# ChristodoulosPappas/IPLS-Java-API

Hardware: AMD Instinct MI355X
Metric: aggregated-gradient GB/s (device-resident), 32 peers×4M doubles/partition (higher is better)
Workload: dtype f64

## Files before the change

### include/ipls_agg.h

```cpp
#ifndef IPLS_AGG_H
#define IPLS_AGG_H

#include <stddef.h>
#include <stdint.h>

#ifdef __cplusplus
extern "C" {
#endif

#define IPLS_AGG_ABI_VERSION 4

#define IPLS_OK           0
#define IPLS_E_INVAL     -1
#define IPLS_E_RANGE     -2
#define IPLS_E_NEGSIZE   -3
#define IPLS_E_NOMEM     -4
#define IPLS_E_DEVICE    -5
#define IPLS_E_FORMAT    -6
#define IPLS_E_NODEV     -7

#define IPLS_TGT_AGG      0
#define IPLS_TGT_REP      1
#define IPLS_TGT_WEIGHTS  2
#define IPLS_TGT_WADDR    3
// ... 180 lines not shown
#define IPLS_KERNEL_REDUCE        1
#define IPLS_KERNEL_ROUND         2
#define IPLS_KERNEL_FOLD1         3
#define IPLS_KERNEL_REDUCE_SCALAR 4
#define IPLS_KERNEL_REDUCE_F32    5
#define IPLS_KERNEL_REDUCE_H16    6
#define IPLS_KERNEL_ROUND_F32     7
#define IPLS_KERNEL_ROUND_H16     8
#define IPLS_KERNEL_FOLD1_F32     9
#define IPLS_KERNEL_FOLD1_H16    10
#define IPLS_KERNEL_UPDATE_FLAT  11
#define IPLS_SHAPE_BIG    1
#define IPLS_SHAPE_MID    2
#define IPLS_SHAPE_SMALL  3
#define IPLS_SHAPE_HALF   4
typedef struct ipls_launch_info {
    int32_t kernel, shape, block, vectors, seqf, map;
    int64_t grid;
    int32_t be_in, be_out, start;
    int32_t staged;
} ipls_launch_info;
int ipls_agg_last_launch(ipls_agg *h, ipls_launch_info *out);


int ipls_host_alloc(size_t bytes, void **ptr);
int ipls_host_free(void *ptr);


int ipls_synth_fill(void *dst, int64_t len, uint64_t seed, int p, int k, int dst_kind,
                    void *stream);

int ipls_checksum_dev(const void *src, int64_t n, int src_kind, uint64_t *out, void *stream);

int ipls_encode_secure(const void *src, void *dst, int64_t n, int src_kind, int dst_kind,
                       void *stream);

int64_t ipls_frame_parse(const uint8_t *frame, int64_t len, int16_t *pid, int32_t *a,
                         int32_t *b, int64_t *payload_off, int64_t *origin_off);

int64_t ipls_frame_encode(const double *g, int64_t n, int g_kind, int32_t a, int32_t b,
                          int16_t pid, const uint8_t *origin, int32_t origin_len,
                          uint8_t *out, int64_t out_cap);


int64_t ipls_pair_parse(const uint8_t *buf, int64_t len, int32_t *workers, int64_t *payload_off);

// ... 35 lines not shown
```

### ipls-java-api_amd/csrc/engine.hip

```cpp
#include <hip/hip_runtime.h>

#include <algorithm>
#include <atomic>
#include <cstdarg>
#include <cstdio>
#include <cstdlib>
#include <cstring>
#include <deque>
#include <map>
#include <memory>
#include <mutex>
#include <new>
#include <set>
#include <string>
#include <thread>
#include <vector>

#include "../../include/ipls_agg.h"
#include "ipls_kernels.hpp"
#include "javaser.hpp"
#include "engine.hpp"
#include "pubsub_host.hpp"

using namespace ipls;
// ... 30 lines not shown
  hipEvent_t free_ev = nullptr;
  bool free_pending = false;
};

struct ipls_dev {
  std::mutex mu;
  std::string err;
  int device = 0;
  hipStream_t stream = nullptr;

  int64_t model_size = 0;
  int P = 0;
  int64_t chunk = 0;
  int secure = 0;
  std::vector<int64_t> len, flat_off;
  int64_t max_len = 0, flat_total = 0;
  int p_lo = 0;
  int64_t flat_base = 0;

  double* arena = nullptr;
  int64_t arena_elems = 0;
  std::vector<int64_t> agg_off, rep_off, w_off, fut_off;
  std::vector<uint8_t> agg_zero, rep_zero, fut_zero;

  PinnedSlot ring[kRingSlots];
  void* d_table[kRingSlots] = {};
  size_t d_table_cap[kRingSlots] = {};
  int ring_next = 0;
  std::vector<unsigned char> last_table;
  int last_slot = -1;

  std::mutex stage_mu;
  std::vector<ipls_stage*> stage_all, stage_idle;
  void* d_scratch = nullptr;
  size_t scratch_bytes = 0;
  hipEvent_t copy_ev = nullptr;
  static constexpr int kCopyThreads = 4;
  hipStream_t copy_stream[kCopyThreads] = {};
  hipEvent_t ingest_ev = nullptr;
  std::vector<hipEvent_t> msg_ev;
  struct StageSlot {
    void* d = nullptr;
    size_t cap = 0;
    hipEvent_t free_ev = nullptr;
    bool pending = false;
  };
// ... 66 lines not shown
int check_part(ipls_dev* h, int p) {
  if (p < 0 || p >= h->P) return fail(h, IPLS_E_RANGE, "partition %d out of range [0,%d)", p, h->P);
  return IPLS_OK;
}

int64_t target_off(ipls_dev* h, int p, int target) {
  switch (target) {
    case IPLS_TGT_AGG: return h->agg_off[p];
    case IPLS_TGT_REP: return h->rep_off[p];
    case IPLS_TGT_WEIGHTS:
    case IPLS_TGT_WADDR: return h->w_off[p];
    case IPLS_TGT_FUTURE: return h->fut_off[p];
    default: return -1;
  }
}

uint8_t* zero_flag(ipls_dev* h, int p, int target) {
  if (target == IPLS_TGT_AGG) return &h->agg_zero[p];
  if (target == IPLS_TGT_REP) return &h->rep_zero[p];
  if (target == IPLS_TGT_FUTURE) return &h->fut_zero[p];
  return nullptr;
}

int materialize(ipls_dev* h, int p, int target) {
  uint8_t* f = zero_flag(h, p, target);
  if (f && *f) {
    HIP_TRY(h, hipMemsetAsync(h->arena + target_off(h, p, target), 0, (size_t)h->len[p] * 8, h->stream));
    *f = 0;
  }
  return IPLS_OK;
}

int ensure_pinned(ipls_dev* h, PinnedSlot& s, size_t bytes) {
  if (s.pending) {
    HIP_TRY(h, hipEventSynchronize(s.ev));
    s.pending = false;
  }
  if (s.cap < bytes) {
    if (s.host) HIP_TRY(h, hipHostFree(s.host));
    s.host = nullptr;
    s.cap = 0;
    size_t cap = std::max<size_t>(bytes, 64 << 10);
    HIP_TRY(h, hipHostMalloc(&s.host, cap, hipHostMallocDefault));
    s.cap = cap;
  }
  if (!s.ev) HIP_TRY(h, hipEventCreateWithFlags(&s.ev, hipEventDisableTiming));
  return IPLS_OK;
}

int fail_nl(ipls_dev* h, int code, const char* fmt, ...) {
  char buf[512];
// ... 535 lines not shown
    if (nz == n_parts) start = IPLS_START_ZERO;
    else if (nz) {
      for (int q = 0; q < n_parts; ++q) {
        int rc = materialize(h, p_first + q, target);
        if (rc) return rc;
      }
    }
  }
  if (!fin && !tr_in && n_parts == 1 && k == 1 && bufs[0]) {
    unsigned long long* d0 = dst_of(0);
    const int64_t L = len_of(0);
    if (d0 && !((uintptr_t)bufs[0] & 15) && !((uintptr_t)d0 & 15) && L > 0) {
      const auto* s0 = (const unsigned long long*)bufs[0];
      const unsigned blocks =
          std::max(1u, std::min<unsigned>(blocks_for((L >> 1), kBlock * 4), host_src ? 128u : 4096u));
#define F1(BI, BO, ST) hipLaunchKernelGGL((k_fold1<BI, BO, ST>), dim3(blocks), dim3(kBlock), 0, h->stream, d0, s0, L)
#define F1S(BI, BO) do { if (start == kZero) F1(BI, BO, kZero); else if (start == kFirst) F1(BI, BO, kFirst); else F1(BI, BO, kAccum); } while (0)
      if (be_in) { if (be_out) F1S(true, true); else F1S(true, false); }
      else { if (be_out) F1S(false, true); else F1S(false, false); }
#undef F1S
#undef F1
      HIP_TRY(h, hipGetLastError());
      h->last_launch = launch_info(IPLS_KERNEL_FOLD1, 0, kBlock, 4, 0, 0, blocks, be_in, be_out, kstart(start));
      if (!ext_dst)
        if (uint8_t* f = zero_flag(h, p_first, target)) *f = 0;
      return IPLS_OK;
    }
  }
  if (!fin && tr_in && arrival && !be_out && start != IPLS_START_FIRST && n_parts == 1 && k == 1 && bufs[0]) {
    unsigned long long* d0 = dst_of(0);
    const int64_t L = len_of(0);
    if (d0 && !((uintptr_t)bufs[0] & (uintptr_t)(4 * fmt_size(fmt_in) - 1)) && !((uintptr_t)d0 & 15) && L > 0) {
      const unsigned blocks = std::max(1u, std::min<unsigned>(blocks_for(L >> 2, kBlock * kFold1NarrowR), kFold1NarrowGrid));
      with_narrow(fmt_in, [&](auto s) {
        typedef decltype(s) S;
        const auto* s0 = (const typename S::elem*)bufs[0];
        if (start == IPLS_START_ZERO)
          hipLaunchKernelGGL((k_fold1_narrow<S, kZero, kFold1NarrowR>), dim3(blocks), dim3(kBlock), 0, h->stream, d0, s0, L);
        else
          hipLaunchKernelGGL((k_fold1_narrow<S, kAccum, kFold1NarrowR>), dim3(blocks), dim3(kBlock), 0, h->stream, d0, s0, L);
      });
      HIP_TRY(h, hipGetLastError());
      h->last_launch = launch_info(fmt_size(fmt_in) == 4 ? IPLS_KERNEL_FOLD1_F32 : IPLS_KERNEL_FOLD1_H16, 0, kBlock,
                                   kFold1NarrowR, 1, 0, blocks, false, false, kstart(start));
      if (!ext_dst)
        if (uint8_t* f = zero_flag(h, p_first, target)) *f = 0;
      return IPLS_OK;
    }
  }
  bool aligned16 = true;
  int64_t maxL = 0;
  for (int q = 0; q < n_parts; ++q) maxL = std::max(maxL, len_of(q));
  for (int64_t i = 0; i < (int64_t)n_parts * k; ++i) {
    if (!bufs[i]) return fail(h, IPLS_E_INVAL, "bucket pointer %lld is NULL", (long long)i);
    uintptr_t a = (uintptr_t)bufs[i];
    if (a & (uintptr_t)(fmt_size(fmt_in) - 1))
      return fail(h, IPLS_E_INVAL, "bucket %lld not %d-byte aligned", (long long)i, fmt_size(fmt_in));
    if (a & 15) aligned16 = false;
  }
  const size_t desc_bytes = sizeof(PartDesc) * n_parts;
  const size_t bytes = desc_bytes + sizeof(void*) * (size_t)n_parts * k;
  std::vector<unsigned char> tbl(bytes);
  PartDesc* pd = (PartDesc*)tbl.data();
  for (int q = 0; q < n_parts; ++q) {
    const int p = p_first + q;
    pd[q].len = len_of(q);
    pd[q].dst = dst_of(q);
    pd[q].init = pd[q].dst;
    pd[q].rep = nullptr;
// ... 31 lines not shown
    }
    HIP_TRY(h, hipGetLastError());
    for (int q = p_first; q < p_first + n_parts; ++q) h->agg_zero[q] = h->rep_zero[q] = 1;
    return IPLS_OK;
  }
  if (tr_in) {
    h->last_launch = with_narrow(fmt_in, [&](auto s) {
      typedef decltype(s) S;
      return launch_reduce_narrow<S>(be_out, kstart(start), aligned16, maxL, n_parts, h->stream,
                                     (const typename S::elem* const*)dbufs, dparts, k);
    });
  } else if (aligned16) {
    h->last_launch = launch_reduce(be_in, be_out, start, maxL, n_parts, h->stream, dbufs, dparts, k);
  } else {
    const int64_t tile = (int64_t)kBlock * 8;
    const int tpp = (int)((maxL + tile - 1) / tile);
    launch_reduce_scalar(be_in, be_out, start, dim3((unsigned)tpp * n_parts), h->stream, dbufs, dparts, k, tpp,
                         tile);
    h->last_launch = launch_info(IPLS_KERNEL_REDUCE_SCALAR, 0, kBlock, 1, 0, 0, (int64_t)tpp * n_parts, be_in, be_out,
                                 kstart(start));
  }
  HIP_TRY(h, hipGetLastError());
  if (!ext_dst)
    for (int q = 0; q < n_parts; ++q) {
      uint8_t* f = zero_flag(h, p_first + q, target);
      if (f) *f = 0;
    }
  return IPLS_OK;
}

int partition_geometry(const ipls_agg_cfg* c, std::vector<int64_t>& len, std::vector<int64_t>& off,
                       int64_t& chunk, std::string& why) {
  const int P = c->n_partitions;
  len.resize(P);
  off.resize(P);
  if (c->model_size > 0) {
    chunk = ref_chunk(c->model_size, P);
    for (int i = 0; i < P; ++i) {
      int64_t L = ((int64_t)(i + 1) * chunk > c->model_size) ? c->model_size - (int64_t)i * chunk + 1
                                                             : chunk + 1;
      if (L < 1) {
        char b[160];
        snprintf(b, sizeof b, "partition %d length %lld < 1 (%s)", i, (long long)L,
                 L < 0 ? "NegativeArraySizeException, IPLS.java:1863"
                       : "ArrayIndexOutOfBoundsException, IPLS.java:1894");
        why = b;
        return L < 0 ? IPLS_E_NEGSIZE : IPLS_E_RANGE;
      }
      len[i] = L;
      off[i] = (int64_t)i * chunk;
// ... 52 lines not shown
  if (!h) return fail(nullptr, IPLS_E_NOMEM, "host allocation failed");
  std::string why;
  std::vector<int64_t> glen, goff;
  int rc = partition_geometry(cfg, glen, goff, h->chunk, why);
  if (rc) {
    delete h;
    return fail(nullptr, rc, "%s", why.c_str());
  }
  h->len.assign(glen.begin() + p_lo, glen.begin() + p_hi);
  h->flat_off.assign(goff.begin() + p_lo, goff.begin() + p_hi);
  h->p_lo = p_lo;
  h->flat_base = p_hi > p_lo ? h->flat_off[0] : 0;
  h->P = p_hi - p_lo;
  h->device = device;
  h->model_size = cfg->model_size;
  h->secure = cfg->secure;
  h->agg_off.resize(h->P);
  h->rep_off.resize(h->P);
  h->w_off.resize(h->P);
  h->fut_off.resize(h->P);
  h->agg_zero.assign(h->P, 1);
  h->rep_zero.assign(h->P, 1);
  h->fut_zero.assign(h->P, 1);
  int64_t cur = 0;
  for (int p = 0; p < h->P; ++p) {
    h->max_len = std::max(h->max_len, h->len[p]);
    h->flat_total = std::max(h->flat_total, h->flat_off[p] + h->len[p] - 1);
    h->agg_off[p] = cur; cur = align_up(cur + h->len[p], kAlignElems);
    h->rep_off[p] = cur; cur = align_up(cur + h->len[p], kAlignElems);
    h->w_off[p] = cur;   cur = align_up(cur + h->len[p], kAlignElems);
    h->fut_off[p] = cur; cur = align_up(cur + h->len[p], kAlignElems);
  }
  h->arena_elems = cur;
  h->gbuf_len = h->model_size > 0 ? (int64_t)((int32_t)h->model_size / cfg->n_partitions) + 2 : cfg->bucket_len;
  auto cleanup = [&](int code) {
    (void)hipGetLastError();
    dev_close(h);
    return code;
  };
  if (dev_use(h->device) != hipSuccess) return cleanup(fail(nullptr, IPLS_E_DEVICE, "dev_use(%d) failed", h->device));
  if (hipStreamCreateWithFlags(&h->stream, hipStreamNonBlocking) != hipSuccess)
    return cleanup(fail(nullptr, IPLS_E_DEVICE, "hipStreamCreate failed"));
  if (h->arena_elems > 0 && hipMalloc(&h->arena, (size_t)h->arena_elems * 8) != hipSuccess) {
    (void)hipGetLastError();
    h->arena = nullptr;
    return cleanup(fail(nullptr, IPLS_E_NOMEM, "hipMalloc of %lld-byte arena failed", (long long)h->arena_elems * 8));
// ... 569 lines not shown
            const flat_job& f = fj[j0 + j];
            if (f.q < 0 || f.q >= h->P || f.ncopy < 0 || f.ncopy > h->len[f.q] - 1 || f.lo < 0)
              return fail(h, IPLS_E_INVAL, "internal: bad whole-gradient job");
            FlatJob& o = jobs[(size_t)j];
            o.lo = f.lo;
            o.ncopy = f.ncopy;
            o.L = h->len[f.q];
            o.dst = (unsigned long long*)(h->arena + h->agg_off[f.q]);
            o.zero = h->agg_zero[f.q];
            maxL = std::max(maxL, o.L);
            all_vec = all_vec && f.ncopy >= tile;
            all_zero = all_zero && o.zero;
          }
          void* djobs = nullptr;
          if (int r = upload_table(h, jobs.data(), jobs.size() * sizeof(FlatJob), &djobs)) return r;
          const dim3 grid(blocks_for(maxL, tile), (unsigned)nj);
          if (fmt == kFmtF64) launch_update_flat<FmtD64, false>(h->stream, grid, (const FlatJob*)djobs, d_in);
          else if (fmt == kFmtBE) launch_update_flat<FmtD64, true>(h->stream, grid, (const FlatJob*)djobs, d_in);
          else
            with_narrow(fmt, [&](auto sfmt) {
              launch_update_flat<decltype(sfmt), false>(h->stream, grid, (const FlatJob*)djobs, d_in);
            });
          HIP_TRY(h, hipGetLastError());
          for (int j = 0; j < nj; ++j) h->agg_zero[fj[j0 + j].q] = 0;
          h->last_launch = launch_info(IPLS_KERNEL_UPDATE_FLAT, 0, kBlock, kFlatR, all_vec ? 1 : 0, 0,
                                       (int64_t)grid.x * grid.y, fmt == kFmtBE, false, all_zero ? kZero : kAccum);
        }
      }
      return IPLS_OK;
    }();
  }
  for (int s = 0; s < n; ++s) {
    ipls_dev* h = c[s].h;
    ipls_stage* st = c[s].st;
    if (dev_use(h->device) == hipSuccess && hipEventRecord(st->free_ev, h->stream) == hipSuccess) {
      st->free_pending = true;
    } else {
      (void)hipGetLastError();
      (void)hipStreamSynchronize(h->stream);
      st->free_pending = false;
    }
  }
  for (int s = n - 1; s >= 0; --s) c[s].h->mu.unlock();
  for (int s = 0; s < n; ++s) {
    if (rc) {
      (void)dev_use(c[s].h->device);
      for (int i = 0; i < c[s].st->n_copy; ++i) (void)hipStreamSynchronize(c[s].st->copy[i]);
// ... 155 lines not shown
int dev_reset(ipls_dev* h, int p) {
  if (!h) return fail(nullptr, IPLS_E_INVAL, "null handle");
  IPLS_LOCK(h);
  if (p == IPLS_ALL_PARTITIONS) {
    for (int q = 0; q < h->P; ++q) h->agg_zero[q] = h->rep_zero[q] = 1;
    return IPLS_OK;
  }
  if (int rc = check_part(h, p)) return rc;
  h->agg_zero[p] = h->rep_zero[p] = 1;
  return IPLS_OK;
}

int dev_promote_future(ipls_dev* h, const int32_t* parts, int n_parts) {
  if (!h) return fail(nullptr, IPLS_E_INVAL, "null handle");
  IPLS_LOCK(h);
  if (n_parts < 0 || (n_parts > 0 && !parts)) return fail(h, IPLS_E_INVAL, "bad partition list");
  for (int i = 0; i < n_parts; ++i)
    if (int rc = check_part(h, parts[i])) return rc;
  for (int i = 0; i < n_parts; ++i) {
    const int p = parts[i];
    std::swap(h->agg_off[p], h->fut_off[p]);
    h->agg_zero[p] = h->fut_zero[p];
    h->fut_zero[p] = 1;
  }
  return IPLS_OK;
}

int dev_device_ptr(ipls_dev* h, int p, int target, void** ptr) {
  if (!h || !ptr) return fail(h, IPLS_E_INVAL, "null argument");
  IPLS_LOCK(h);
  if (int rc = check_part(h, p)) return rc;
  if (target_off(h, p, target) < 0) return fail(h, IPLS_E_INVAL, "bad target %d", target);
  HIP_TRY(h, dev_use(h->device));
  if (int rc = materialize(h, p, target)) return rc;
  *ptr = h->arena + target_off(h, p, target);
  return IPLS_OK;
}

int dev_read(ipls_dev* h, int p, int target, void* dst, int64_t n, int dst_kind) {
  if (!h || !dst) return fail(h, IPLS_E_INVAL, "null argument");
  IPLS_LOCK(h);
  if (int rc = check_part(h, p)) return rc;
  if (target_off(h, p, target) < 0) return fail(h, IPLS_E_INVAL, "bad target %d", target);
  const int64_t L = h->len[p];
  if (n < L) return fail(h, IPLS_E_RANGE, "output of %lld < partition length %lld", (long long)n, (long long)L);
  HIP_TRY(h, dev_use(h->device));
  if (int rc = materialize(h, p, target)) return rc;
  const double* srcd = h->arena + target_off(h, p, target);
  switch (dst_kind) {
    case IPLS_HOST_F64:
      return d2h(h, dst, srcd, (size_t)L * 8);
    case IPLS_DEV_F64:
      HIP_TRY(h, hipMemcpyAsync(dst, srcd, (size_t)L * 8, hipMemcpyDeviceToDevice, h->stream));
      return IPLS_OK;
    case IPLS_DEV_BE:
      launch_bswap(h->stream, (const unsigned long long*)srcd, (unsigned long long*)dst, L);
      HIP_TRY(h, hipGetLastError());
      return IPLS_OK;
// ... 8 lines not shown
  }
}

int dev_checksum(ipls_dev* h, int p, int target, uint64_t* out) {
  if (!h || !out) return fail(h, IPLS_E_INVAL, "null argument");
  IPLS_LOCK(h);
  if (int rc = check_part(h, p)) return rc;
  if (target_off(h, p, target) < 0) return fail(h, IPLS_E_INVAL, "bad target %d", target);
  HIP_TRY(h, dev_use(h->device));
  if (int rc = materialize(h, p, target)) return rc;
  HIP_TRY(h, hipMemsetAsync(h->d_sum, 0, 8, h->stream));
  const int64_t L = h->len[p];
  hipLaunchKernelGGL(k_checksum<false>, dim3(std::max(1u, std::min<unsigned>(blocks_for(L, kBlock * 8), 2048))),
                     dim3(kBlock), 0, h->stream,
                     (const unsigned long long*)(h->arena + target_off(h, p, target)), L, h->d_sum);
  HIP_TRY(h, hipGetLastError());
  unsigned long long v = 0;
  if (int rc = d2h(h, &v, h->d_sum, 8)) return rc;
  *out = v;
  return IPLS_OK;
}

static int finalize_range(ipls_dev* h, int p0, int np) {
  bool rep_zero_all = true;
  for (int q = p0; q < p0 + np; ++q) {
    if (int rc = materialize(h, q, IPLS_TGT_AGG)) return rc;
    rep_zero_all = rep_zero_all && h->rep_zero[q];
  }
  if (!rep_zero_all)
    for (int q = p0; q < p0 + np; ++q)
      if (int rc = materialize(h, q, IPLS_TGT_REP)) return rc;
  std::vector<FinDesc> fd(np);
  int64_t maxL = 0;
  for (int q = 0; q < np; ++q) {
    fd[q] = FinDesc{h->len[p0 + q], h->agg_off[p0 + q], h->rep_off[p0 + q], h->w_off[p0 + q]};
    maxL = std::max(maxL, fd[q].len);
  }
  void* dtab = nullptr;
  if (int rc = upload_table(h, fd.data(), fd.size() * sizeof(FinDesc), &dtab)) return rc;
  const int64_t tile = kFinTile;
  const int tpp = (int)((maxL + tile - 1) / tile);
  if (rep_zero_all)
    hipLaunchKernelGGL((k_finalize<true, false>), dim3((unsigned)tpp * np), dim3(kBlock), 0, h->stream,
                       (const FinDesc*)dtab, h->arena, tpp);
  else
    hipLaunchKernelGGL((k_finalize<false, false>), dim3((unsigned)tpp * np), dim3(kBlock), 0, h->stream,
                       (const FinDesc*)dtab, h->arena, tpp);
  HIP_TRY(h, hipGetLastError());
  for (int q = p0; q < p0 + np; ++q) h->agg_zero[q] = h->rep_zero[q] = 1;
  return IPLS_OK;
}

static int divide_range(ipls_dev* h, int p0, int np, unsigned long long* d_out, bool be) {
  std::vector<DivDesc> dd(np);
  int64_t maxn = 0;
  for (int q = 0; q < np; ++q) {
    const int p = p0 + q;
    dd[q] = DivDesc{h->len[p], h->w_off[p], h->flat_off[p] - h->flat_off[p0]};
    maxn = std::max(maxn, h->len[p] - 1);
  }
  if (maxn <= 0) return IPLS_OK;
  void* dtab = nullptr;
  if (int rc = upload_table(h, dd.data(), dd.size() * sizeof(DivDesc), &dtab)) return rc;
  const int64_t tile = kDivTile;
  const int tpp = (int)((maxn + tile - 1) / tile);
  const dim3 g((unsigned)tpp * np);
#define DIV(B, S) hipLaunchKernelGGL((k_divide<B, S>), g, dim3(kBlock), 0, h->stream, (const DivDesc*)dtab, (const double*)h->arena, d_out, tpp)
  if (be) { if (h->secure) DIV(true, true); else DIV(true, false); }
  else { if (h->secure) DIV(false, true); else DIV(false, false); }
#undef DIV
  HIP_TRY(h, hipGetLastError());
  return IPLS_OK;
// ... 484 lines not shown
    const bool vec = al16((const char*)d + esz * lo) && al16(acc);
    const dim3 g = vec ? dim3(std::max(1u, blocks_for(L, kEwTile))) : dim3(blocks_for(L, kBlock));
#define UPD(BI, M)                                                                                              \
  do {                                                                                                          \
    if (vec) hipLaunchKernelGGL((k_split<BI, false, M, true>), g, dim3(kBlock), 0, h->stream, d, lo, nc[p], L, acc); \
    else hipLaunchKernelGGL((k_split<BI, false, M, false>), g, dim3(kBlock), 0, h->stream, d, lo, nc[p], L, acc); \
  } while (0)
#define UPDN(M)                                                                                                 \
  do {                                                                                                          \
    if (vec) hipLaunchKernelGGL((k_split_narrow<S, false, M, true>), g, dim3(kBlock), 0, h->stream, (const typename S::elem*)d, lo, nc[p], L, acc); \
    else hipLaunchKernelGGL((k_split_narrow<S, false, M, false>), g, dim3(kBlock), 0, h->stream, (const typename S::elem*)d, lo, nc[p], L, acc); \
  } while (0)
    if (fmt_trainer(fmt))
      with_narrow(fmt, [&](auto s) {
        typedef decltype(s) S;
        if (zero) UPDN(2);
        else UPDN(1);
      });
    else if (be) { if (zero) UPD(true, 2); else UPD(true, 1); }
    else { if (zero) UPD(false, 2); else UPD(false, 1); }
#undef UPDN
#undef UPD
    HIP_TRY(h, hipGetLastError());
    h->agg_zero[p] = 0;
  }
  return IPLS_OK;
}

int dev_get_partitions(ipls_dev* h, void* out, int64_t n, int out_kind) {
  if (!h || !out) return fail(h, IPLS_E_INVAL, "null argument");
  IPLS_LOCK(h);
  const int64_t M = h->flat_total - h->flat_base;
  if (n < M) return fail(h, IPLS_E_RANGE, "output of %lld < model size %lld", (long long)n, (long long)M);
  if (out_kind != IPLS_HOST_F64 && out_kind != IPLS_HOST_BE_CANON && out_kind != IPLS_DEV_F64 &&
      !kind_trainer(out_kind))
    return fail(h, IPLS_E_INVAL, "bad out_kind %d", out_kind);
  HIP_TRY(h, dev_use(h->device));
  if (kind_trainer(out_kind)) {
    const Fmt fmt = kind_fmt(out_kind);
    const int esz = fmt_size(fmt);
    if ((uintptr_t)out & (uintptr_t)(esz - 1)) return fail(h, IPLS_E_INVAL, "output not %d-byte aligned", esz);
    void* d_n = out;
    if (kind_trainer_host(out_kind)) {
      if (int rc = ensure_scratch(h, (size_t)std::max<int64_t>(M, 1) * esz)) return rc;
      d_n = h->d_scratch;
    }
    if (int rc = divide_range_narrow(h, 0, h->P, d_n, fmt)) return rc;
// ... 368 lines not shown
  HIP_TRY(h, dev_use(h->device));
  const void* d = src;
  bool be = src_kind == IPLS_HOST_BE || src_kind == IPLS_DEV_BE;
  if (src_kind == IPLS_HOST_F64 || src_kind == IPLS_HOST_BE) {
    if (int rc = ensure_scratch(h, (size_t)L * 8)) return rc;
    if (int rc = stage_h2d(h, h->d_scratch, src, (size_t)L * 8)) return rc;
    d = h->d_scratch;
  } else if (src_kind != IPLS_DEV_F64 && src_kind != IPLS_DEV_BE) {
    return fail(h, IPLS_E_INVAL, "bad src_kind %d", src_kind);
  }
  if (int rc = materialize(h, p, target)) return rc;
  double* t = h->arena + target_off(h, p, target);
  const bool vec = al16(t) && al16(d);
  const dim3 g = ew_grid(L, vec, 8192);
  auto gs = (const unsigned long long*)d;
  if (be) {
    if (vec) hipLaunchKernelGGL((k_blend<true, true>), g, dim3(kBlock), 0, h->stream, t, gs, L, a, b);
    else hipLaunchKernelGGL((k_blend<true, false>), g, dim3(kBlock), 0, h->stream, t, gs, L, a, b);
  } else {
    if (vec) hipLaunchKernelGGL((k_blend<false, true>), g, dim3(kBlock), 0, h->stream, t, gs, L, a, b);
    else hipLaunchKernelGGL((k_blend<false, false>), g, dim3(kBlock), 0, h->stream, t, gs, L, a, b);
  }
  HIP_TRY(h, hipGetLastError());
  return IPLS_OK;
}

int dev_scale(ipls_dev* h, int p, int dst_target, int src_target, double c) {
  if (!h) return fail(nullptr, IPLS_E_INVAL, "null handle");
  IPLS_LOCK(h);
  if (int rc = check_part(h, p)) return rc;
  if (target_off(h, p, dst_target) < 0 || target_off(h, p, src_target) < 0) return fail(h, IPLS_E_INVAL, "bad target");
  HIP_TRY(h, dev_use(h->device));
  if (int rc = materialize(h, p, src_target)) return rc;
  if (uint8_t* f = zero_flag(h, p, dst_target)) *f = 0;
  const int64_t L = h->len[p];
  double* sd = h->arena + target_off(h, p, dst_target);
  auto ss = (const double*)(h->arena + target_off(h, p, src_target));
  if (al16(sd) && al16(ss))
    hipLaunchKernelGGL(k_scale<true>, ew_grid(L, true, 8192), dim3(kBlock), 0, h->stream, sd, ss, L, c);
  else
    hipLaunchKernelGGL(k_scale<false>, ew_grid(L, false, 8192), dim3(kBlock), 0, h->stream, sd, ss, L, c);
  HIP_TRY(h, hipGetLastError());
  return IPLS_OK;
}

int ipls_encode_secure(const void* src, void* dst, int64_t n, int src_kind, int dst_kind, void* stream) {
  if (!src || !dst || n < 0) return fail(nullptr, IPLS_E_INVAL, "bad argument");
  if ((src_kind != IPLS_DEV_F64 && src_kind != IPLS_DEV_BE) || (dst_kind != IPLS_DEV_F64 && dst_kind != IPLS_DEV_BE))
    return fail(nullptr, IPLS_E_INVAL, "device operands only (DEV_F64 / DEV_BE)");
  if (n == 0) return IPLS_OK;
  hipStream_t st = (hipStream_t)stream;
  auto s = (const unsigned long long*)src;
  auto d = (unsigned long long*)dst;
  const bool bi = src_kind == IPLS_DEV_BE, bo = dst_kind == IPLS_DEV_BE;
  const bool vec = al16(s) && al16(d);
  const dim3 g = ew_grid(n, vec, 8192);
#define ENC(BI, BO)                                                                                     \
// ... 513 lines not shown
    if (sink(ctx, (const uint8_t*)host, base + o, len) == 0) return IPLS_OK;
    return fail_nl(h, IPLS_E_INVAL, "the byte sink stopped the transfer at offset %lld", (long long)(base + o));
  });
}

int dev_ser_apply(ipls_dev* h, const uint8_t* bytes, int64_t lo, int64_t hi, const int* q, const int64_t* offs, int n,
                  int mode, int target, double a, double b) {
  if (!h || !bytes || !q || !offs || n <= 0 || n > 65535 || lo < 0 || hi < lo) return fail(h, IPLS_E_INVAL, "bad argument");
  IPLS_LOCK(h);
  std::vector<SerApplyJob> jobs((size_t)n);
  int64_t max_pairs = 1;
  for (int i = 0; i < n; ++i) {
    if (int rc = check_part(h, q[i])) return rc;
    if (target_off(h, q[i], target) < 0) return fail(h, IPLS_E_INVAL, "bad target %d", target);
    const int64_t L = h->len[q[i]];
    if (offs[i] < lo || offs[i] + 8 * L > hi) return fail(h, IPLS_E_RANGE, "payload of partition %d outside the file", q[i]);
    jobs[(size_t)i] = SerApplyJob{h->arena + target_off(h, q[i], target), L, offs[i] - lo};
    max_pairs = std::max(max_pairs, L / 2 + 1);
  }
  HIP_TRY(h, dev_use(h->device));
  if (int rc = ensure_scratch(h, (size_t)(hi - lo) + 32)) return rc;
  if (int rc = stage_h2d(h, h->d_scratch, bytes + lo, (size_t)(hi - lo))) return rc;
  for (int i = 0; i < n; ++i) {
    if (mode == IPLS_SAVED_BLEND) {
      if (int rc = materialize(h, q[i], target)) return rc;
    } else if (uint8_t* zf = zero_flag(h, q[i], target)) {
      *zf = 0;
    }
  }
  void* djobs = nullptr;
  if (int rc = upload_table(h, jobs.data(), jobs.size() * sizeof(SerApplyJob), &djobs)) return rc;
  const dim3 grid(std::max(1u, std::min<unsigned>(blocks_for(max_pairs, kSerTileWords), 16384)), (unsigned)n);
  if (mode == IPLS_SAVED_BLEND)
    hipLaunchKernelGGL(k_ser_apply<true>, grid, dim3(kBlock), 0, h->stream, (const SerApplyJob*)djobs,
                       (const unsigned char*)h->d_scratch, a, b);
  else
    hipLaunchKernelGGL(k_ser_apply<false>, grid, dim3(kBlock), 0, h->stream, (const SerApplyJob*)djobs,
                       (const unsigned char*)h->d_scratch, a, b);
  HIP_TRY(h, hipGetLastError());
  return IPLS_OK;
}

int dev_load_dlist(ipls_dev* h, const uint8_t* bytes, int64_t nvals, int64_t hi, bool apply) {
  if (!h || !bytes) return fail(h, IPLS_E_INVAL, "null argument");
  IPLS_LOCK(h);
  const int64_t g0 = h->flat_base;
  if (hi < 0) hi = h->flat_total;
  if (hi > nvals || hi < h->flat_total || g0 > hi)
    return fail(h, IPLS_E_RANGE, "model of %lld values < model size %lld", (long long)nvals, (long long)h->flat_total);
  HIP_TRY(h, dev_use(h->device));
  const int64_t img = 14 * (hi - g0), val_off = align_up(img + 32, 16), flag_off = val_off + 8 * (hi - g0);
// ... 9 lines not shown
  unsigned flag = 0;
  if (int rc = d2h(h, &flag, dflag, 4)) return rc;
  if (flag) return fail(h, IPLS_E_FORMAT, "serialised ArrayList<Double>: an element is not a Double");
  if (!apply) return IPLS_OK;
  for (int p = 0; p < h->P; ++p) {
    const int64_t L = h->len[p];
    hipLaunchKernelGGL(k_load_model<false>, dim3(blocks_for(L, kBlock)), dim3(kBlock), 0, h->stream, vals,
                       h->flat_off[p] - h->flat_base, L - 1, L, h->arena + h->w_off[p]);
    HIP_TRY(h, hipGetLastError());
    h->agg_zero[p] = h->rep_zero[p] = h->fut_zero[p] = 1;
  }
  HIP_TRY(h, hipStreamSynchronize(h->stream));
  return IPLS_OK;
}

int dev_device(const ipls_dev* h) { return h ? h->device : -1; }

int dev_last_launch(const ipls_dev* h, ipls_launch_info* out) {
  if (!h || !out) return IPLS_E_INVAL;
  *out = h->last_launch;
  return IPLS_OK;
}

int dev_reduce_ext(ipls_dev* h, int n, const int64_t* lens, const void* const* bufs, int k, bool be_in,
                   int start_mode, void* const* dst) {
  if (!h) return fail(nullptr, IPLS_E_INVAL, "null handle");
  IPLS_LOCK(h);
  HIP_TRY(h, dev_use(h->device));
  return reduce_dev(h, 0, n, bufs, k, be_fmt(be_in), start_mode, IPLS_TGT_AGG, dst, false, nullptr, false, lens);
}

int dev_other_check(ipls_dev* h) {
  if (!h) return fail(nullptr, IPLS_E_INVAL, "null handle");
  std::lock_guard<std::mutex> lk(h->mu);
  for (auto& kv : h->other)
    if (kv.second.n > h->len[kv.first.first])
      return fail(h, IPLS_E_RANGE, "stored replica of %lld doubles > partition %d length %lld "
                  "(ArrayIndexOutOfBoundsException, IPLS.java:1225)", (long long)kv.second.n,
                  kv.first.first + h->p_lo, (long long)h->len[kv.first.first]);
  return IPLS_OK;
}
```

### ipls-java-api_amd/csrc/engine.hpp

```cpp
#pragma once

#include <stdint.h>

#include <string>
#include <vector>

#include <hip/hip_runtime_api.h>

#include "../../include/ipls_agg.h"

struct ipls_dev;
struct ipls_stage;

enum Fmt : int { kFmtF64 = 0, kFmtBE = 1, kFmtF32 = 2, kFmtF16 = 3, kFmtBF16 = 4 };
constexpr Fmt be_fmt(bool be) { return be ? kFmtBE : kFmtF64; }
constexpr bool fmt_trainer(Fmt f) { return f >= kFmtF32; }
constexpr bool fmt_h16(Fmt f) { return f == kFmtF16 || f == kFmtBF16; }
constexpr int fmt_size(Fmt f) { return f == kFmtF32 ? 4 : fmt_h16(f) ? 2 : 8; }
constexpr Fmt kind_fmt(int kind) {
  return kind == IPLS_DEV_BE || kind == IPLS_HOST_BE                ? kFmtBE
         : kind == IPLS_DEV_F32 || kind == IPLS_HOST_F32            ? kFmtF32
         : kind == IPLS_DEV_F16 || kind == IPLS_HOST_F16            ? kFmtF16
         : kind == IPLS_DEV_BF16 || kind == IPLS_HOST_BF16          ? kFmtBF16
                                                                    : kFmtF64;
}
constexpr bool kind_trainer_dev(int kind) { return kind == IPLS_DEV_F32 || kind == IPLS_DEV_F16 || kind == IPLS_DEV_BF16; }
constexpr bool kind_trainer_host(int kind) { return kind == IPLS_HOST_F32 || kind == IPLS_HOST_F16 || kind == IPLS_HOST_BF16; }
constexpr bool kind_trainer(int kind) { return kind_trainer_dev(kind) || kind_trainer_host(kind); }

const char* dev_last_error(const ipls_dev* h);
void dev_set_thread_error(const char* msg);
hipError_t dev_use(int device);
void dev_track(int device);
int dev_tracked();
int dev_geometry(const ipls_agg_cfg* cfg, std::vector<int64_t>& len, std::vector<int64_t>& off, int64_t& chunk,
                 std::string& why);
int dev_open(const ipls_agg_cfg* cfg, int device, int p_lo, int p_hi, ipls_dev** out);
int dev_close(ipls_dev* h);
int dev_device(const ipls_dev* h);
void* dev_stream(ipls_dev* h);
int dev_sync(ipls_dev* h);
int dev_wait(ipls_dev* h, uint64_t ticket);
int dev_flush(ipls_dev* h);
int dev_set_coalesce(ipls_dev* h, int max_group);
int dev_last_launch(const ipls_dev* h, ipls_launch_info* out);

int dev_load_model(ipls_dev* h, const void* src, int64_t n, int src_kind);
int dev_split(ipls_dev* h, const void* flat, int64_t n, int src_kind, int p, void* dst, int dst_kind);
int dev_update_gradient(ipls_dev* h, const void* flat, int64_t n, int src_kind, const int32_t* owned, int n_owned);
int dev_accumulate(ipls_dev* h, int p, int target, const void* src, int64_t n, int src_kind);
int dev_accumulate_async(ipls_dev* h, int p, int target, const void* src, int64_t n, int src_kind, uint64_t* ticket);
int dev_accumulate_range(ipls_dev* h, int p, int target, const void* src, int64_t off, int64_t n, int src_kind,
                         uint64_t* ticket);
int dev_read_range(ipls_dev* h, int p, int target, void* dst, int64_t off, int64_t n, int dst_kind, uint64_t* ticket);
int dev_accumulate_chunked(ipls_dev* h, int p, int target, int64_t n, int src_kind, int64_t chunk,
                           ipls_chunk_source source, void* ctx);
int dev_accumulate_chunked_narrow(ipls_dev* h, int p, int target, int64_t n, int src_kind, int64_t chunk,
                                  ipls_chunk_source source, void* ctx);
struct flat_job {
  int q;
  int64_t lo, ncopy;
};
struct flat_commit {
  ipls_dev* h;
  ipls_stage* st;
  const flat_job* jobs;
  const int* launch_len;
  int n_launches;
// ... 63 lines not shown
```

### ipls-java-api_amd/csrc/ipls_agg.cpp

```cpp
#include <hip/hip_runtime_api.h>

#include <algorithm>
#include <atomic>
#include <condition_variable>
#include <cstdarg>
#include <cstdio>
#include <cstdlib>
#include <cstring>
#include <deque>
#include <exception>
#include <functional>
#include <map>
#include <memory>
#include <mutex>
#include <new>
#include <string>
#include <thread>
#include <vector>

#include "../../include/ipls_agg.h"
#include "engine.hpp"
#include "flat_plan.hpp"
#include "java_hashmap.hpp"
#include "javaser.hpp"
// ... 415 lines not shown

int ipls_agg_flush(ipls_agg* H) {
  KeepDevice keep_device;
  if (!H) return ferr(nullptr, IPLS_E_INVAL, "null handle");
  for (int s = 0; s < H->S(); ++s)
    if (int rc = fwd(H, s, dev_flush(H->sh[s]))) return rc;
  return IPLS_OK;
}

int ipls_agg_set_coalesce(ipls_agg* H, int max_group) {
  KeepDevice keep_device;
  if (!H) return ferr(nullptr, IPLS_E_INVAL, "null handle");
  for (int s = 0; s < H->S(); ++s)
    if (int rc = fwd(H, s, dev_set_coalesce(H->sh[s], max_group))) return rc;
  return IPLS_OK;
}

int ipls_agg_last_launch(ipls_agg* H, ipls_launch_info* out) {
  KeepDevice keep_device;
  if (!H || !out) return ferr(H, IPLS_E_INVAL, "null argument");
  const int rc = dev_last_launch(H->sh[H->last_shard.load(std::memory_order_relaxed)], out);
  out->staged = H->last_staged.load(std::memory_order_relaxed);
  return rc;
}

int ipls_agg_load_model(ipls_agg* H, const void* src, int64_t n, int src_kind) {
  KeepDevice keep_device;
  if (!H || !src) return ferr(H, IPLS_E_INVAL, "null argument");
  if (src_kind == IPLS_HOST_DLIST) {
    const char* why = nullptr;
    const int64_t nv = ipls::javaser::parse_dlist((const uint8_t*)src, n, &why);
    if (nv < 0) return ferr(H, IPLS_E_FORMAT, "serialised ArrayList<Double>: %s (ObjectInputStream)", why ? why : "malformed");
    if (nv < H->flat_total)
      return ferr(H, IPLS_E_RANGE, "model of %lld values < model size %lld", (long long)nv, (long long)H->flat_total);
    const std::vector<int> ss = nonempty_shards(H);
    auto upto = [&](int s) { return s == ss.back() ? nv : (int64_t)-1; };
    if (ss.size() > 1)
      if (int rc = par_shards(H, ss, [&](int s) { return dev_load_dlist(H->sh[s], (const uint8_t*)src, nv, upto(s), false); }))
        return rc;
    return par_shards(H, ss, [&](int s) { return dev_load_dlist(H->sh[s], (const uint8_t*)src, nv, upto(s), true); });
  }
  if (H->S() == 1) return fwd(H, 0, dev_load_model(H->sh[0], src, n, src_kind));
  if (n < H->flat_total)
    return ferr(H, IPLS_E_RANGE, "model of %lld values < model size %lld", (long long)n, (long long)H->flat_total);
  return par_shards(H, nonempty_shards(H), [&](int s) { return dev_load_model(H->sh[s], src, n, src_kind); });
}
// ... 1113 lines not shown
```

### ipls-java-api_amd/ipls/_native.py

```python
from __future__ import annotations

import ctypes
import os
from pathlib import Path

PKG_ROOT = Path(__file__).resolve().parent.parent
LIB_PATH = Path(os.environ.get("IPLS_AGG_LIB", PKG_ROOT / "lib" / "libipls_agg.so"))
HEADER = PKG_ROOT.parent / "include" / "ipls_agg.h"

IPLS_OK = 0
IPLS_E_INVAL, IPLS_E_RANGE, IPLS_E_NEGSIZE, IPLS_E_NOMEM = -1, -2, -3, -4
IPLS_E_DEVICE, IPLS_E_FORMAT, IPLS_E_NODEV = -5, -6, -7

TGT_AGG, TGT_REP, TGT_WEIGHTS, TGT_WADDR, TGT_FUTURE = 0, 1, 2, 3, 4
HOST_F64, HOST_BE, HOST_FRAME, DEV_F64, DEV_BE, HOST_BE_CANON, HOST_PAIR = 0, 1, 2, 3, 4, 5, 6
HOST_TEXT, DEV_TEXT = 7, 8
HOST_DARR, HOST_DLIST = 9, 10
DEV_F32, HOST_F32 = 11, 12
DEV_F16, HOST_F16, DEV_BF16, HOST_BF16 = 13, 14, 15, 16
SAVED_SET, SAVED_BLEND = 0, 1
KERNEL_REDUCE, KERNEL_ROUND, KERNEL_FOLD1, KERNEL_REDUCE_SCALAR = 1, 2, 3, 4
KERNEL_REDUCE_F32 = 5
KERNEL_REDUCE_H16 = 6
KERNEL_ROUND_F32, KERNEL_ROUND_H16 = 7, 8
# ... 103 lines not shown
    "ipls_agg_reset": (_i, [_vp, _i]),
    "ipls_agg_device_ptr": (_i, [_vp, _i, _i, _P(_vp)]),
    "ipls_agg_stream": (_vp, [_vp]),
    "ipls_agg_sync": (_i, [_vp]),
    "ipls_agg_checksum": (_i, [_vp, _i, _i, _P(_u64)]),
    "ipls_host_alloc": (_i, [ctypes.c_size_t, _P(_vp)]),
    "ipls_host_free": (_i, [_vp]),
    "ipls_synth_fill": (_i, [_vp, _i64, _u64, _i, _i, _i, _vp]),
    "ipls_checksum_dev": (_i, [_vp, _i64, _i, _P(_u64), _vp]),
    "ipls_encode_secure": (_i, [_vp, _vp, _i64, _i, _i, _vp]),
    "ipls_frame_parse": (_i64, [_vp, _i64, _P(_i16), _P(_i32), _P(_i32), _P(_i64), _P(_i64)]),
    "ipls_frame_encode": (_i64, [_vp, _i64, _i, _i32, _i32, _i16, _vp, _i32, _vp, _i64]),
    "ipls_pair_parse": (_i64, [_vp, _i64, _P(_i32), _P(_i64)]),
    "ipls_pair_encode": (_i64, [_i32, _vp, _i64, _i, _vp, _i64]),
    "ipls_agg_commit_partial": (_i64, [_vp, _i, _i32, _vp, _i64]),
    "ipls_agg_merge_files": (_i64, [_vp, _P(_vp), _P(_i64), _i, _i, _vp, _i64]),
    "ipls_agg_partition_device": (_i, [_vp, _i, _P(_i32), _P(_vp)]),
    "ipls_shard_plan": (_i, [_i32, _i32, _P(_i32)]),
    "ipls_agg_reduce_partial": (_i, [_vp, _i, _i, _i, _P(_vp), _i, _i, _i]),
    "ipls_agg_combine_partials": (_i, [_vp, _i, _i]),
    "ipls_agg_publish_partial": (_i64, [_vp, _i, _i, _i32, _i32, _i16, _vp, _i32, _vp, _i64, _i]),
    "ipls_agg_publish_partials": (_i64, [_vp, _vp, _i, _i, _i32, _vp, _i16, _vp, _i32, _vp, _i64, _i, _vp, _vp]),
    "ipls_agg_last_launch": (_i, [_vp, _P(LaunchInfo)]),
    "ipls_saved_parse": (_i64, [_vp, _i64, _P(_i32), _P(_i64), _P(_i64), _i64]),
    "ipls_saved_encode": (_i64, [_P(_i32), _i, _P(_vp), _P(_i64), _i, _vp, _i64]),
    "ipls_darr_parse": (_i64, [_vp, _i64, _P(_i64)]),
    "ipls_darr_encode": (_i64, [_P(ctypes.c_uint8), _i64, _i, _vp, _i64]),
    "ipls_dlist_parse": (_i64, [_vp, _i64, _P(ctypes.c_double), _i64]),
    "ipls_dlist_encode": (_i64, [_P(ctypes.c_uint8), _i64, _i, _vp, _i64]),
    "ipls_agg_save_model": (_i64, [_vp, _P(_i32), _i, _i, _vp, _i64]),
    "ipls_agg_save_model_chunked": (_i, [_vp, _P(_i32), _i, _i, _i64, _vp, _vp]),
    "ipls_agg_save_partition": (_i64, [_vp, _i, _i, _vp, _i64]),
    "ipls_agg_save_model_list": (_i64, [_vp, _i, _vp, _i64]),
    "ipls_agg_load_saved": (_i, [_vp, _vp, _i64, _i, _i, _P(_i32), _i, ctypes.c_double, ctypes.c_double, _P(_i32)]),
}

_lib = None


def load(path) -> ctypes.CDLL:
    if not Path(path).exists():
        raise ImportError(
            f"{path} not found: build it with `make -C ipls-java-api_amd` "
            "(or __graft_entry__.build()); the aggregator has no CPU fallback")
    L = ctypes.CDLL(str(path))
    for name, (res, args) in SIGNATURES.items():
        fn = getattr(L, name)
        fn.restype = res
        fn.argtypes = args
    return L


def lib() -> ctypes.CDLL:
    global _lib
    if _lib is None:
        _lib = load(LIB_PATH)
    return _lib


_fast = None


def fast():
    global _fast
    if _fast is None:
        _fast = False
        if LIB_PATH == PKG_ROOT / "lib" / "libipls_agg.so":
            try:
                from . import _fast as m
            except ImportError:
# ... 55 lines not shown
```

### ipls-java-api_amd/ipls/aggregator.py

```python
from __future__ import annotations

import ctypes
from dataclasses import dataclass

import numpy as np

from . import _native as N


@dataclass
class DeviceBuffer:
    ptr: int
    n: int
    big_endian: bool = False
    dtype: str = "f64"

    def __post_init__(self):
        if self.dtype not in ("f64", "f32", "half", "bf16"):
            raise ValueError(f"dtype must be 'f64', 'f32', 'half' or 'bf16', not {self.dtype!r}")
        if self.dtype != "f64" and self.big_endian:
            raise ValueError(f"big-endian buffers hold doubles: dtype={self.dtype!r} cannot be big_endian")

    @classmethod
    def from_tensor(cls, t, big_endian: bool = False) -> "DeviceBuffer":
# ... 694 lines not shown
        total = self._chk(self._lib.ipls_agg_publish_partials(
            self._h, parts.ctypes.data, n, target, a, bb.ctypes.data, pid, op, o.size, None, 0, N.HOST_TEXT,
            lens.ctypes.data, offs.ctypes.data))
        if out is not None:
            if isinstance(out, PinnedBuffer):
                ptr, cap, kind = out.ptr, out.nbytes, N.HOST_TEXT
            else:
                (ptr, cap), kind = self._device_text_out(out, out_cap, total), N.DEV_TEXT
            self._chk(self._lib.ipls_agg_publish_partials(
                self._h, parts.ctypes.data, n, target, a, bb.ctypes.data, pid, op, o.size, ptr, cap, kind,
                None, None))
            return lens[:n].tolist(), offs[:n].tolist()
        buf = np.empty(max(1, total), dtype=np.uint8)
        self._chk(self._lib.ipls_agg_publish_partials(
            self._h, parts.ctypes.data, n, target, a, bb.ctypes.data, pid, op, o.size, buf.ctypes.data, total,
            N.HOST_TEXT, None, None))
        return [buf[offs[i]:offs[i] + lens[i]].tobytes() for i in range(n)]

    def last_launch(self) -> dict:
        li = N.LaunchInfo()
        self._chk(self._lib.ipls_agg_last_launch(self._h, ctypes.byref(li)))
        return {f: getattr(li, f) for f, _ in N.LaunchInfo._fields_}

    def read(self, partition: int, target: int = N.TGT_AGG, *, big_endian: bool = False):
        L = self.lengths[partition]
        if big_endian:
            buf = np.empty(8 * L, dtype=np.uint8)
            self._chk(self._lib.ipls_agg_read(self._h, partition, target, buf.ctypes.data, L, N.HOST_BE))
            return buf.tobytes()
        buf = np.empty(L)
        self._chk(self._lib.ipls_agg_read(self._h, partition, target, buf.ctypes.data, L, N.HOST_F64))
        return buf

    def reset(self, partition: int = N.ALL_PARTITIONS):
        self._chk(self._lib.ipls_agg_reset(self._h, partition))

    def device_ptr(self, partition: int, target: int = N.TGT_AGG) -> int:
        p = ctypes.c_void_p()
        self._chk(self._lib.ipls_agg_device_ptr(self._h, partition, target, ctypes.byref(p)))
        return int(p.value)

    def checksum(self, partition: int, target: int = N.TGT_AGG) -> int:
        v = ctypes.c_uint64()
        self._chk(self._lib.ipls_agg_checksum(self._h, partition, target, ctypes.byref(v)))
        return int(v.value)

# ... 156 lines not shown
```

Before: 7045.

## Finalize by swapping aggregate and weight buffers when aggregate is canonical

Tracks per-partition state flags for whether the aggregate buffer holds a clean sum started from zero and whether its pointer was handed out. When replicas are empty and the aggregate is canonical and not lent, finalize swaps the aggregate and weight offsets instead of running the finalize kernel over the data. The kernel runs only for the remaining partitions. This removes a full read/write pass over the partitions it skips, but adds state-tracking complexity and a correctness risk if any write path fails to update the flags.

```diff
diff --git a/include/ipls_agg.h b/include/ipls_agg.h
--- a/include/ipls_agg.h
+++ b/include/ipls_agg.h
@@ -226,6 +226,8 @@
 } ipls_launch_info;
 int ipls_agg_last_launch(ipls_agg *h, ipls_launch_info *out);
 
+int ipls_agg_finalize_stats(ipls_agg *h, int64_t *swapped, int64_t *by_kernel);
+
 
 int ipls_host_alloc(size_t bytes, void **ptr);
 int ipls_host_free(void *ptr);
diff --git a/ipls-java-api_amd/csrc/engine.hip b/ipls-java-api_amd/csrc/engine.hip
--- a/ipls-java-api_amd/csrc/engine.hip
+++ b/ipls-java-api_amd/csrc/engine.hip
@@ -76,6 +76,10 @@
   int64_t arena_elems = 0;
   std::vector<int64_t> agg_off, rep_off, w_off, fut_off;
   std::vector<uint8_t> agg_zero, rep_zero, fut_zero;
+  std::vector<uint8_t> agg_canon, fut_canon;
+  std::vector<uint8_t> agg_lent, fut_lent;
+  bool fin_swap = true;
+  int64_t fin_swapped = 0, fin_by_kernel = 0;
 
   PinnedSlot ring[kRingSlots];
   void* d_table[kRingSlots] = {};
@@ -188,11 +192,35 @@
   return nullptr;
 }
 
+uint8_t* canon_flag(ipls_dev* h, int p, int target) {
+  if (target == IPLS_TGT_AGG) return &h->agg_canon[p];
+  if (target == IPLS_TGT_FUTURE) return &h->fut_canon[p];
+  return nullptr;
+}
+
+enum Wrote { kWroteRaw, kWroteSum, kWroteFresh };
+
+void note_write(ipls_dev* h, int p, int target, Wrote how) {
+  uint8_t* z = zero_flag(h, p, target);
+  const bool was_zero = z && *z;
+  if (z) *z = 0;
+  if (uint8_t* c = canon_flag(h, p, target)) {
+    if (how == kWroteFresh) *c = 1;
+    else if (how == kWroteRaw || was_zero) *c = 0;
+  }
+}
+
+Wrote wrote_by_fold(int start, bool be_out) {
+  if (be_out || start == IPLS_START_FIRST) return kWroteRaw;
+  return start == IPLS_START_ZERO ? kWroteFresh : kWroteSum;
+}
+
 int materialize(ipls_dev* h, int p, int target) {
   uint8_t* f = zero_flag(h, p, target);
   if (f && *f) {
     HIP_TRY(h, hipMemsetAsync(h->arena + target_off(h, p, target), 0, (size_t)h->len[p] * 8, h->stream));
     *f = 0;
+    if (uint8_t* c = canon_flag(h, p, target)) *c = 1;
   }
   return IPLS_OK;
 }
@@ -774,8 +802,7 @@
 #undef F1
       HIP_TRY(h, hipGetLastError());
       h->last_launch = launch_info(IPLS_KERNEL_FOLD1, 0, kBlock, 4, 0, 0, blocks, be_in, be_out, kstart(start));
-      if (!ext_dst)
-        if (uint8_t* f = zero_flag(h, p_first, target)) *f = 0;
+      if (!ext_dst) note_write(h, p_first, target, wrote_by_fold(start, be_out));
       return IPLS_OK;
     }
   }
@@ -795,8 +822,7 @@
       HIP_TRY(h, hipGetLastError());
       h->last_launch = launch_info(fmt_size(fmt_in) == 4 ? IPLS_KERNEL_FOLD1_F32 : IPLS_KERNEL_FOLD1_H16, 0, kBlock,
                                    kFold1NarrowR, 1, 0, blocks, false, false, kstart(start));
-      if (!ext_dst)
-        if (uint8_t* f = zero_flag(h, p_first, target)) *f = 0;
+      if (!ext_dst) note_write(h, p_first, target, wrote_by_fold(start, be_out));
       return IPLS_OK;
     }
   }
@@ -874,10 +900,7 @@
   }
   HIP_TRY(h, hipGetLastError());
   if (!ext_dst)
-    for (int q = 0; q < n_parts; ++q) {
-      uint8_t* f = zero_flag(h, p_first + q, target);
-      if (f) *f = 0;
-    }
+    for (int q = 0; q < n_parts; ++q) note_write(h, p_first + q, target, wrote_by_fold(start, be_out));
   return IPLS_OK;
 }
 
@@ -976,6 +999,12 @@
   h->agg_zero.assign(h->P, 1);
   h->rep_zero.assign(h->P, 1);
   h->fut_zero.assign(h->P, 1);
+  h->agg_canon.assign(h->P, 1);
+  h->fut_canon.assign(h->P, 1);
+  h->agg_lent.assign(h->P, 0);
+  h->fut_lent.assign(h->P, 0);
+  const char* fs = std::getenv("IPLS_FINALIZE_SWAP");
+  h->fin_swap = !(fs && fs[0] == '0');
   int64_t cur = 0;
   for (int p = 0; p < h->P; ++p) {
     h->max_len = std::max(h->max_len, h->len[p]);
@@ -1591,7 +1620,8 @@
               launch_update_flat<decltype(sfmt), false>(h->stream, grid, (const FlatJob*)djobs, d_in);
             });
           HIP_TRY(h, hipGetLastError());
-          for (int j = 0; j < nj; ++j) h->agg_zero[fj[j0 + j].q] = 0;
+          for (int j = 0; j < nj; ++j)
+            note_write(h, fj[j0 + j].q, IPLS_TGT_AGG, jobs[(size_t)j].zero ? kWroteFresh : kWroteSum);
           h->last_launch = launch_info(IPLS_KERNEL_UPDATE_FLAT, 0, kBlock, kFlatR, all_vec ? 1 : 0, 0,
                                        (int64_t)grid.x * grid.y, fmt == kFmtBE, false, all_zero ? kZero : kAccum);
         }
@@ -1793,6 +1823,8 @@
     std::swap(h->agg_off[p], h->fut_off[p]);
     h->agg_zero[p] = h->fut_zero[p];
     h->fut_zero[p] = 1;
+    std::swap(h->agg_canon[p], h->fut_canon[p]);
+    std::swap(h->agg_lent[p], h->fut_lent[p]);
   }
   return IPLS_OK;
 }
@@ -1805,6 +1837,8 @@
   HIP_TRY(h, dev_use(h->device));
   if (int rc = materialize(h, p, target)) return rc;
   *ptr = h->arena + target_off(h, p, target);
+  if (target == IPLS_TGT_AGG) h->agg_lent[p] = 1;
+  if (target == IPLS_TGT_FUTURE) h->fut_lent[p] = 1;
   return IPLS_OK;
 }
 
@@ -1859,32 +1893,50 @@
 }
 
 static int finalize_range(ipls_dev* h, int p0, int np) {
-  bool rep_zero_all = true;
+  std::vector<int> rest;
+  rest.reserve(np);
+  for (int q = p0; q < p0 + np; ++q)
+    if (!(h->fin_swap && h->rep_zero[q] && !h->agg_zero[q] && h->agg_canon[q] && !h->agg_lent[q])) rest.push_back(q);
+  if (!rest.empty()) {
+    bool rep_zero_all = true;
+    for (int q : rest) {
+      if (int rc = materialize(h, q, IPLS_TGT_AGG)) return rc;
+      rep_zero_all = rep_zero_all && h->rep_zero[q];
+    }
+    if (!rep_zero_all)
+      for (int q : rest)
+        if (int rc = materialize(h, q, IPLS_TGT_REP)) return rc;
+    const int nr = (int)rest.size();
+    std::vector<FinDesc> fd(nr);
+    int64_t maxL = 0;
+    for (int i = 0; i < nr; ++i) {
+      const int q = rest[i];
+      fd[i] = FinDesc{h->len[q], h->agg_off[q], h->rep_off[q], h->w_off[q]};
+      maxL = std::max(maxL, fd[i].len);
+    }
+    void* dtab = nullptr;
+    if (int rc = upload_table(h, fd.data(), fd.size() * sizeof(FinDesc), &dtab)) return rc;
+    const int64_t tile = kFinTile;
+    const int tpp = (int)((maxL + tile - 1) / tile);
+    if (rep_zero_all)
+      hipLaunchKernelGGL((k_finalize<true, false>), dim3((unsigned)tpp * nr), dim3(kBlock), 0, h->stream,
+                         (const FinDesc*)dtab, h->arena, tpp);
+    else
+      hipLaunchKernelGGL((k_finalize<false, false>), dim3((unsigned)tpp * nr), dim3(kBlock), 0, h->stream,
+                         (const FinDesc*)dtab, h->arena, tpp);
+    HIP_TRY(h, hipGetLastError());
+  }
+  size_t r = 0;
   for (int q = p0; q < p0 + np; ++q) {
-    if (int rc = materialize(h, q, IPLS_TGT_AGG)) return rc;
-    rep_zero_all = rep_zero_all && h->rep_zero[q];
-  }
-  if (!rep_zero_all)
-    for (int q = p0; q < p0 + np; ++q)
-      if (int rc = materialize(h, q, IPLS_TGT_REP)) return rc;
-  std::vector<FinDesc> fd(np);
-  int64_t maxL = 0;
-  for (int q = 0; q < np; ++q) {
-    fd[q] = FinDesc{h->len[p0 + q], h->agg_off[p0 + q], h->rep_off[p0 + q], h->w_off[p0 + q]};
-    maxL = std::max(maxL, fd[q].len);
-  }
-  void* dtab = nullptr;
-  if (int rc = upload_table(h, fd.data(), fd.size() * sizeof(FinDesc), &dtab)) return rc;
-  const int64_t tile = kFinTile;
-  const int tpp = (int)((maxL + tile - 1) / tile);
-  if (rep_zero_all)
-    hipLaunchKernelGGL((k_finalize<true, false>), dim3((unsigned)tpp * np), dim3(kBlock), 0, h->stream,
-                       (const FinDesc*)dtab, h->arena, tpp);
-  else
-    hipLaunchKernelGGL((k_finalize<false, false>), dim3((unsigned)tpp * np), dim3(kBlock), 0, h->stream,
-                       (const FinDesc*)dtab, h->arena, tpp);
-  HIP_TRY(h, hipGetLastError());
-  for (int q = p0; q < p0 + np; ++q) h->agg_zero[q] = h->rep_zero[q] = 1;
+    if (r < rest.size() && rest[r] == q) {
+      ++r;
+      ++h->fin_by_kernel;
+    } else {
+      std::swap(h->agg_off[q], h->w_off[q]);
+      ++h->fin_swapped;
+    }
+    h->agg_zero[q] = h->rep_zero[q] = 1;
+  }
   return IPLS_OK;
 }
 
@@ -2415,7 +2467,7 @@
 #undef UPDN
 #undef UPD
     HIP_TRY(h, hipGetLastError());
-    h->agg_zero[p] = 0;
+    note_write(h, p, IPLS_TGT_AGG, zero ? kWroteFresh : kWroteSum);
   }
   return IPLS_OK;
 }
@@ -2830,6 +2882,7 @@
     else hipLaunchKernelGGL((k_blend<false, false>), g, dim3(kBlock), 0, h->stream, t, gs, L, a, b);
   }
   HIP_TRY(h, hipGetLastError());
+  note_write(h, p, target, kWroteRaw);
   return IPLS_OK;
 }
 
@@ -2840,7 +2893,7 @@
   if (target_off(h, p, dst_target) < 0 || target_off(h, p, src_target) < 0) return fail(h, IPLS_E_INVAL, "bad target");
   HIP_TRY(h, dev_use(h->device));
   if (int rc = materialize(h, p, src_target)) return rc;
-  if (uint8_t* f = zero_flag(h, p, dst_target)) *f = 0;
+  note_write(h, p, dst_target, kWroteRaw);
   const int64_t L = h->len[p];
   double* sd = h->arena + target_off(h, p, dst_target);
   auto ss = (const double*)(h->arena + target_off(h, p, src_target));
@@ -3400,11 +3453,9 @@
   if (int rc = ensure_scratch(h, (size_t)(hi - lo) + 32)) return rc;
   if (int rc = stage_h2d(h, h->d_scratch, bytes + lo, (size_t)(hi - lo))) return rc;
   for (int i = 0; i < n; ++i) {
-    if (mode == IPLS_SAVED_BLEND) {
+    if (mode == IPLS_SAVED_BLEND)
       if (int rc = materialize(h, q[i], target)) return rc;
-    } else if (uint8_t* zf = zero_flag(h, q[i], target)) {
-      *zf = 0;
-    }
+    note_write(h, q[i], target, kWroteRaw);
   }
   void* djobs = nullptr;
   if (int rc = upload_table(h, jobs.data(), jobs.size() * sizeof(SerApplyJob), &djobs)) return rc;
@@ -3460,6 +3511,14 @@
   return IPLS_OK;
 }
 
+int dev_finalize_stats(ipls_dev* h, int64_t* swapped, int64_t* by_kernel) {
+  if (!h || !swapped || !by_kernel) return IPLS_E_INVAL;
+  std::lock_guard<std::mutex> lk(h->mu);
+  *swapped = h->fin_swapped;
+  *by_kernel = h->fin_by_kernel;
+  return IPLS_OK;
+}
+
 int dev_reduce_ext(ipls_dev* h, int n, const int64_t* lens, const void* const* bufs, int k, bool be_in,
                    int start_mode, void* const* dst) {
   if (!h) return fail(nullptr, IPLS_E_INVAL, "null handle");
diff --git a/ipls-java-api_amd/csrc/engine.hpp b/ipls-java-api_amd/csrc/engine.hpp
--- a/ipls-java-api_amd/csrc/engine.hpp
+++ b/ipls-java-api_amd/csrc/engine.hpp
@@ -44,6 +44,7 @@
 int dev_flush(ipls_dev* h);
 int dev_set_coalesce(ipls_dev* h, int max_group);
 int dev_last_launch(const ipls_dev* h, ipls_launch_info* out);
+int dev_finalize_stats(ipls_dev* h, int64_t* swapped, int64_t* by_kernel);
 
 int dev_load_model(ipls_dev* h, const void* src, int64_t n, int src_kind);
 int dev_split(ipls_dev* h, const void* flat, int64_t n, int src_kind, int p, void* dst, int dst_kind);
diff --git a/ipls-java-api_amd/csrc/ipls_agg.cpp b/ipls-java-api_amd/csrc/ipls_agg.cpp
--- a/ipls-java-api_amd/csrc/ipls_agg.cpp
+++ b/ipls-java-api_amd/csrc/ipls_agg.cpp
@@ -461,6 +461,18 @@
   const int rc = dev_last_launch(H->sh[H->last_shard.load(std::memory_order_relaxed)], out);
   out->staged = H->last_staged.load(std::memory_order_relaxed);
   return rc;
+}
+
+int ipls_agg_finalize_stats(ipls_agg* H, int64_t* swapped, int64_t* by_kernel) {
+  if (!H || !swapped || !by_kernel) return ferr(H, IPLS_E_INVAL, "null argument");
+  *swapped = *by_kernel = 0;
+  for (int s = 0; s < H->S(); ++s) {
+    int64_t a = 0, b = 0;
+    if (int rc = dev_finalize_stats(H->sh[s], &a, &b)) return ferr(H, rc, "null shard");
+    *swapped += a;
+    *by_kernel += b;
+  }
+  return IPLS_OK;
 }
 
 int ipls_agg_load_model(ipls_agg* H, const void* src, int64_t n, int src_kind) {
diff --git a/ipls-java-api_amd/ipls/_native.py b/ipls-java-api_amd/ipls/_native.py
--- a/ipls-java-api_amd/ipls/_native.py
+++ b/ipls-java-api_amd/ipls/_native.py
@@ -149,6 +149,7 @@
     "ipls_agg_publish_partial": (_i64, [_vp, _i, _i, _i32, _i32, _i16, _vp, _i32, _vp, _i64, _i]),
     "ipls_agg_publish_partials": (_i64, [_vp, _vp, _i, _i, _i32, _vp, _i16, _vp, _i32, _vp, _i64, _i, _vp, _vp]),
     "ipls_agg_last_launch": (_i, [_vp, _P(LaunchInfo)]),
+    "ipls_agg_finalize_stats": (_i, [_vp, _P(_i64), _P(_i64)]),
     "ipls_saved_parse": (_i64, [_vp, _i64, _P(_i32), _P(_i64), _P(_i64), _i64]),
     "ipls_saved_encode": (_i64, [_P(_i32), _i, _P(_vp), _P(_i64), _i, _vp, _i64]),
     "ipls_darr_parse": (_i64, [_vp, _i64, _P(_i64)]),
@@ -172,7 +173,12 @@
             "(or __graft_entry__.build()); the aggregator has no CPU fallback")
     L = ctypes.CDLL(str(path))
     for name, (res, args) in SIGNATURES.items():
-        fn = getattr(L, name)
+        try:
+            fn = getattr(L, name)
+        except AttributeError:
+            if "IPLS_AGG_LIB" in os.environ:
+                continue
+            raise
         fn.restype = res
         fn.argtypes = args
     return L
diff --git a/ipls-java-api_amd/ipls/aggregator.py b/ipls-java-api_amd/ipls/aggregator.py
--- a/ipls-java-api_amd/ipls/aggregator.py
+++ b/ipls-java-api_amd/ipls/aggregator.py
@@ -740,6 +740,11 @@
         self._chk(self._lib.ipls_agg_last_launch(self._h, ctypes.byref(li)))
         return {f: getattr(li, f) for f, _ in N.LaunchInfo._fields_}
 
+    def finalize_stats(self) -> tuple[int, int]:
+        s, k = ctypes.c_int64(), ctypes.c_int64()
+        self._chk(self._lib.ipls_agg_finalize_stats(self._h, ctypes.byref(s), ctypes.byref(k)))
+        return int(s.value), int(k.value)
+
     def read(self, partition: int, target: int = N.TGT_AGG, *, big_endian: bool = False):
         L = self.lengths[partition]
         if big_endian:
```

Measured after the change: 7061, median of 6. Within noise of the previous version (+0.2%).
